# nerfstudio-project/gsplat

Hardware: AMD Instinct MI355X
Metric: Mpixels/s fwd+bwd @1M Gaussians/1080p (higher is better)
Workload: dtype f32; 1 GPU; c3: 1M synthetic Gaussians, 1x1920x1080, SH deg 3, 16x16 tiles, fwd+bwd; gaussians_per_gpu=1000000, cameras_per_gpu=1, packed=False, parallelism=single

## Files before the change

gsplat_amd/csrc/bitonic64.hpp:

```cpp
#pragma once
#include "common.hpp"

namespace gsx {

constexpr uint64_t kBtPadInt = ~0ull;
constexpr uint64_t kBtPadF64 = 0x7FF0000000000000ull;

__device__ __forceinline__ int bt_phys(int i) { return i + (i >> 3); }
__device__ __forceinline__ int bt_off(int b, int lj)
{
    const int sb = b << lj;
    return sb + (sb >> 3);
}
__device__ __forceinline__ bool bt_key_is_odd(uint32_t depth_bits)
{
    return (depth_bits - 0x00100000u) >= (0x7FF00000u - 0x00100000u);
}

__device__ __forceinline__ void bt_cmpx_int(uint64_t &x, uint64_t &y, bool up)
{
    const bool sw     = (x > y) == up;
    const uint64_t lo = sw ? y : x, hi = sw ? x : y;
    x = lo;
    y = hi;
}
__device__ __forceinline__ void bt_cmpx_int_up(uint64_t &x, uint64_t &y)
{
    const bool sw    = x > y;
    const uint64_t t = sw ? y : x;
    y                = sw ? x : y;
    x                = t;
}

template <int G, int NT>
__device__ __forceinline__ void bt_group_int(uint64_t *s, int P, int lk, int lj, int tid)
{
    constexpr int R = 1 << G;
    for (int t = tid; t < (P >> G); t += NT) {
        const int i = ((t >> lj) << (lj + G)) | (t & ((1 << lj) - 1));
        const uint32_t m32 = 0u - (((uint32_t)i >> lk) & 1u);
        const uint64_t m   = ((uint64_t)m32 << 32) | m32;
        uint64_t *p        = s + bt_phys(i);
        uint64_t e[R];
#pragma unroll
        for (int b = 0; b < R; ++b) e[b] = p[bt_off(b, lj)] ^ m;
#pragma unroll
        for (int q = G - 1; q >= 0; --q)
#pragma unroll
            for (int b = 0; b < R; ++b)
                if (!(b & (1 << q))) bt_cmpx_int_up(e[b], e[b | (1 << q)]);
#pragma unroll
        for (int b = 0; b < R; ++b) p[bt_off(b, lj)] = e[b] ^ m;
    }
}

template <int NT, typename Sync>
__device__ __forceinline__ void bt_sort_int(uint64_t *s, int lp, int tid, Sync &&SYNC)
{
    const int P = 1 << lp;
    for (int t = tid; t < (P >> 3); t += NT) {
        uint64_t *p = s + 9 * t;
        uint64_t e[8];
#pragma unroll
        for (int b = 0; b < 8; ++b) e[b] = p[b];
#pragma unroll
        for (int lk = 1; lk <= 3; ++lk)
#pragma unroll
            for (int q = lk - 1; q >= 0; --q)
#pragma unroll
                for (int b = 0; b < 8; ++b)
                    if (!(b & (1 << q))) {
                        const bool up = lk < 3 ? ((b & (1 << lk)) == 0) : ((t & 1) == 0);
                        bt_cmpx_int(e[b], e[b | (1 << q)], up);
                    }
#pragma unroll
        for (int b = 0; b < 8; ++b) p[b] = e[b];
    }
    SYNC();
    for (int lk = 4; lk <= lp; ++lk) {
        for (int top = lk - 1; top >= 0;) {
            const int gsz = top + 1 < 3 ? top + 1 : 3;
            const int lj  = top - gsz + 1;
            if (gsz == 3) bt_group_int<3, NT>(s, P, lk, lj, tid);
            else if (gsz == 2) bt_group_int<2, NT>(s, P, lk, lj, tid);
            else bt_group_int<1, NT>(s, P, lk, lj, tid);
            SYNC();
            top -= gsz;
        }
    }
}

__device__ __forceinline__ void bt_minmax(double &x, double &y)
{
    double lo, hi;
    asm("v_min_f64 %0, %1, %2" : "=v"(lo) : "v"(x), "v"(y));
    asm("v_max_f64 %0, %1, %2" : "=v"(hi) : "v"(x), "v"(y));
    x = lo;
    y = hi;
}
__device__ __forceinline__ double bt_as_f64(uint64_t w) { return __builtin_bit_cast(double, w); }
__device__ __forceinline__ uint64_t bt_as_u64(double d) { return __builtin_bit_cast(uint64_t, d); }

template <int G, int NT>
__device__ __forceinline__ void bt_group_f64(uint64_t *s, int P, int lk, int lj, int tid)
{
    constexpr int R = 1 << G;
    for (int t = tid; t < (P >> G); t += NT) {
        const int i = ((t >> lj) << (lj + G)) | (t & ((1 << lj) - 1));
        const uint64_t neg = (uint64_t)(((uint32_t)i >> lk) & 1u) << 63;
        uint64_t *p        = s + bt_phys(i);
        double e[R];
#pragma unroll
        for (int b = 0; b < R; ++b) e[b] = bt_as_f64(p[bt_off(b, lj)] ^ neg);
#pragma unroll
        for (int q = G - 1; q >= 0; --q)
#pragma unroll
            for (int b = 0; b < R; ++b)
                if (!(b & (1 << q))) bt_minmax(e[b], e[b | (1 << q)]);
#pragma unroll
        for (int b = 0; b < R; ++b) p[bt_off(b, lj)] = bt_as_u64(e[b]) ^ neg;
    }
}

template <int NT, typename Sync>
__device__ __forceinline__ void bt_sort_f64(uint64_t *s, int lp, int tid, Sync &&SYNC)
{
    const int P = 1 << lp;
    for (int t = tid; t < (P >> 3); t += NT) {
        uint64_t *p = s + 9 * t;
        double e[8];
#pragma unroll
        for (int b = 0; b < 8; ++b) e[b] = bt_as_f64(p[b]);
#pragma unroll
        for (int lk = 1; lk <= 2; ++lk)
#pragma unroll
            for (int q = lk - 1; q >= 0; --q)
#pragma unroll
                for (int b = 0; b < 8; ++b)
                    if (!(b & (1 << q))) {
                        if ((b & (1 << lk)) == 0) bt_minmax(e[b], e[b | (1 << q)]);
                        else bt_minmax(e[b | (1 << q)], e[b]);
                    }
        const uint64_t neg = (uint64_t)((uint32_t)t & 1u) << 63;
#pragma unroll
        for (int b = 0; b < 8; ++b) e[b] = bt_as_f64(bt_as_u64(e[b]) ^ neg);
#pragma unroll
        for (int q = 2; q >= 0; --q)
#pragma unroll
            for (int b = 0; b < 8; ++b)
                if (!(b & (1 << q))) bt_minmax(e[b], e[b | (1 << q)]);
#pragma unroll
        for (int b = 0; b < 8; ++b) p[b] = bt_as_u64(e[b]) ^ neg;
    }
    SYNC();
    for (int lk = 4; lk <= lp; ++lk) {
        for (int top = lk - 1; top >= 0;) {
            const int gsz = top + 1 < 3 ? top + 1 : 3;
            const int lj  = top - gsz + 1;
            if (gsz == 3) bt_group_f64<3, NT>(s, P, lk, lj, tid);
            else if (gsz == 2) bt_group_f64<2, NT>(s, P, lk, lj, tid);
            else bt_group_f64<1, NT>(s, P, lk, lj, tid);
            SYNC();
            top -= gsz;
        }
    }
}

bool bitonic_f64_enabled();

}
```

gsplat_amd/csrc/isect_binned.hip:

```cpp
#include "isect_binwalk.hpp"
#include "bitonic64.hpp"
#include "isect_fused.hpp"
#include <cstdlib>
#include <mutex>
#include <new>

namespace gsx {

constexpr int kRowThreads     = 1024;
constexpr int kBnThreads      = 256;
constexpr int kBnMaxBins      = 16384;
constexpr uint32_t kBnMaxTiles = 36864;

struct BinHeader {
    int32_t overflow;
    int32_t big_count;
    int32_t b_done;
    int32_t pad[5];
};

struct BinGeom {
    int64_t rows, rows_per_image, cap_entries;
    uint32_t n_images, cpi, rpc, n_chunks;
    uint32_t tile_size, tile_w, tile_h, n_tiles;
    uint32_t bw, bh, bins_x, bins_y, n_bins, n_bins_total, tile_bits;
    uint32_t kx, ky;
    int32_t skew_cap;
    int32_t skew_ratio;
};

struct BinBuffers {
    BinHeader *hdr;
    int32_t *table;
    int32_t *bin_count;
    int32_t *unit_count;
    uint4 *unit_rec;
    uint32_t *unit_row;
    int32_t *bin_start;
    uint4 *row_rec;
    uint2 *e_pair;
    uint16_t *e_mask;
    int32_t *tile_count;
    int32_t *big_list;
};

struct BinArgs {
    BinGeom g;
    BinBuffers b;
    const float *means2d;
    const int32_t *radii;
    const float *depths;
    const float *conics;
    const float *opacities;
    const uint8_t *tile_mask;
    int32_t *tiles_per_gauss;
    int32_t *isect_offsets;
    int64_t *n_isects;
    int64_t *max_tile_len;
    uint64_t *keys_out;
    int32_t *vals_out;
    uint2 *bucketed;
    uint32_t dbg;
    uint32_t sort_int;
};

__device__ __forceinline__ void bn_chunk_rows(const BinGeom &g, uint32_t chunk, int64_t &lo, int64_t &hi, uint32_t &img)
{
    img                = chunk / g.cpi;
    const uint32_t sub = chunk % g.cpi;
    lo                 = (int64_t)img * g.rows_per_image + (int64_t)sub * g.rpc;
    hi                 = min(lo + (int64_t)g.rpc, (int64_t)(img + 1) * g.rows_per_image);
}

struct BnRow {
    float mx, my, rx, ry, A, B, C, op;
};
__device__ __forceinline__ BnRow bn_load_row(const BinArgs &a, int64_t r, bool has_conic)
{
    BnRow q;
    const int2 rad = reinterpret_cast<const int2 *>(a.radii)[r];
    const v2f m    = reinterpret_cast<const v2f *>(a.means2d)[r];
    q.rx = (float)rad.x; q.ry = (float)rad.y; q.mx = m.x; q.my = m.y;
    q.A = q.B = q.C = q.op = 0.0f;
    if (has_conic) {
        q.A  = a.conics[3 * r];
        q.B  = a.conics[3 * r + 1];
        q.C  = a.conics[3 * r + 2];
        q.op = a.opacities[r];
    }
    return q;
}
__device__ __forceinline__ WalkPrep bn_prepare(const BnRow &q, bool has_conic, const BinGeom &g)
{
    if (!(q.rx > 0.0f && q.ry > 0.0f)) {
        WalkPrep p{};
        p.any = false;
        return p;
    }
    return walk_prepare(q.mx, q.my, q.rx, q.ry, has_conic, q.A, q.B, q.C, q.op, g.tile_size, g.tile_w, g.tile_h);
}

constexpr uint32_t kRecNone = 0u, kRecSmall = 1u, kRecBig = 2u;
constexpr int kInlineSlabs  = 2;
constexpr int kAPark        = 512;
constexpr int kAQueue       = 2048;
constexpr int kATake        = 128;
constexpr int kParkWords    = 17;
constexpr uint32_t kUnitCap = 1024;

template <bool FIXED>
struct BinShape {
    uint32_t bw, bh, kx, ky;
    __device__ __forceinline__ explicit BinShape(const BinGeom &g)
        : bw(FIXED ? 4u : g.bw), bh(FIXED ? 2u : g.bh), kx(FIXED ? 2u : g.kx), ky(FIXED ? 4u : g.ky) {}
};
template <bool FIXED>
__device__ __forceinline__ uint32_t rec_bin_mask(uint64_t M, const BinShape<FIXED> &sh, uint32_t i, uint32_t j)
{
    return block_bin_mask(M, sh.bw, sh.bh, sh.kx, i, j);
}
template <bool FIXED>
__device__ __forceinline__ uint4 make_record(uint64_t M, uint32_t bbx, uint32_t bby, uint32_t dbits, const BinGeom &g,
                                             const BinShape<FIXED> &sh, int32_t *s_hist)
{
    uint32_t used = 0;
    for (uint32_t j = 0; j < sh.ky; ++j)
        for (uint32_t i = 0; i < sh.kx; ++i)
            if (rec_bin_mask(M, sh, i, j)) {
                used |= 1u << (j * sh.kx + i);
                if (s_hist) atomicAdd(&s_hist[(bby + j) * g.bins_x + bbx + i], 1);
            }
    return make_uint4((uint32_t)M, (uint32_t)(M >> 32), bbx | (bby << 8) | (kRecSmall << 16) | (used << 18), dbits);
}

__device__ __forceinline__ void park_walk(uint32_t *rw, const WalkPrep &p, uint32_t slot, bool one, uint32_t org, uint32_t dbits)
{
    rw[0] = (uint32_t)p.x0 | ((uint32_t)p.y0 << 16); rw[1] = (uint32_t)p.x1 | ((uint32_t)p.y1 << 16);
    rw[2] = slot | (p.ellipse ? 1u << 16 : 0u) | (p.alongY ? 1u << 17 : 0u) | (one ? 1u << 18 : 0u);
    rw[3] = org;
    rw[4] = dbits;
    const float pf[12] = {p.B, p.coeff, p.disc, p.t, p.pu, p.pv, p.bmin_u, p.bmax_u, p.bmin_v, p.bmax_v, p.u_at_vmin, p.u_at_vmax};
#pragma unroll
    for (int k = 0; k < 12; ++k) rw[5 + k] = __float_as_uint(pf[k]);
}
__device__ __forceinline__ WalkPrep parked_walk(const uint32_t *rw)
{
    WalkPrep p;
    p.x0 = (int)(rw[0] & 0xFFFFu); p.y0 = (int)(rw[0] >> 16); p.x1 = (int)(rw[1] & 0xFFFFu); p.y1 = (int)(rw[1] >> 16);
    p.any = true; p.ellipse = (rw[2] >> 16) & 1u; p.alongY = (rw[2] >> 17) & 1u;
    p.B = __uint_as_float(rw[5]); p.coeff = __uint_as_float(rw[6]); p.disc = __uint_as_float(rw[7]);
    p.t = __uint_as_float(rw[8]); p.pu = __uint_as_float(rw[9]); p.pv = __uint_as_float(rw[10]);
    p.bmin_u = __uint_as_float(rw[11]); p.bmax_u = __uint_as_float(rw[12]); p.bmin_v = __uint_as_float(rw[13]);
    p.bmax_v = __uint_as_float(rw[14]); p.u_at_vmin = __uint_as_float(rw[15]); p.u_at_vmax = __uint_as_float(rw[16]);
    return p;
}

template <bool FIXED>
__global__ void __launch_bounds__(kRowThreads) bin_rect_kernel(const BinArgs a)
{
    extern __shared__ int32_t s_hist[];
    __shared__ uint32_t s_q[kAQueue];
    __shared__ uint32_t s_row[kAPark][kParkWords];
    __shared__ int32_t s_tpg[2 * kRowThreads];
    __shared__ int32_t s_qn, s_qlim, s_mn, s_units, s_anybig;
    const BinGeom &g = a.g;
    const BinShape<FIXED> sh(g);
    for (uint32_t i = threadIdx.x; i < g.n_bins; i += kRowThreads) s_hist[i] = 0;
    if (threadIdx.x == 0) {
        s_units = 0; s_mn = 0; s_qn = 0; s_qlim = kAQueue; s_anybig = 0;
        if (blockIdx.x == 0) { a.b.hdr->overflow = 0; a.b.hdr->big_count = 0; a.b.hdr->b_done = 0; }
    }
    int64_t lo, hi;
    uint32_t img;
    bn_chunk_rows(g, blockIdx.x, lo, hi, img);
    const bool has_conic = (a.conics != nullptr) && (a.opacities != nullptr);
    const uint8_t *tmask = a.tile_mask ? a.tile_mask + (size_t)img * g.n_tiles : nullptr;
    const uint32_t W = sh.kx * sh.bw, Hh = sh.ky * sh.bh;
    uint64_t col = 0;
    for (uint32_t y = 0; y < Hh; ++y) col |= 1ull << (y * W);
    uint4 *unit_rec    = a.b.unit_rec + (size_t)blockIdx.x * kUnitCap;
    uint32_t *unit_row = a.b.unit_row + (size_t)blockIdx.x * kUnitCap;
    constexpr int kU = 2;
    for (int64_t base = lo; base < hi; base += kRowThreads * kU) {
        BnRow q[kU];
        uint32_t dbits[kU];
#pragma unroll
        for (int u = 0; u < kU; ++u) {
            const int64_t r = base + u * kRowThreads + threadIdx.x;
            q[u].rx = q[u].ry = 0.0f;
            dbits[u] = 0u;
            if (r < hi) {
                q[u]     = bn_load_row(a, r, has_conic);
                dbits[u] = __float_as_uint(a.depths[r]);
            }
        }
        if (base != lo) {
            __syncthreads();
            if (threadIdx.x == 0) { s_mn = 0; s_qn = 0; s_qlim = kAQueue; s_anybig = 0; }
        }
        __syncthreads();
        uint32_t units[kU], done[kU];
        int32_t ms[kU];
        bool left = false;
#pragma unroll
        for (int u = 0; u < kU; ++u) {
            const int64_t r = base + u * kRowThreads + threadIdx.x;
            units[u] = done[u] = 0u;
            ms[u]    = -1;
            if (r >= hi) continue;
            uint4 rec        = make_uint4(0u, 0u, kRecNone << 16, dbits[u]);
            const WalkPrep p = bn_prepare(q[u], has_conic, g);
            bool now         = true;
            if (p.any) {
                const uint32_t bx0 = (uint32_t)p.x0 / sh.bw, bx1 = ((uint32_t)p.x1 + sh.bw - 1) / sh.bw;
                const uint32_t by0 = (uint32_t)p.y0 / sh.bh, by1 = ((uint32_t)p.y1 + sh.bh - 1) / sh.bh;
                const uint32_t w = bx1 - bx0, h = by1 - by0;
                const bool one   = w <= sh.kx && h <= sh.ky;
                const int slabs  = p.ellipse ? min(p.x1 - p.x0, p.y1 - p.y0) : 1;
                if (one && slabs <= (int)(((a.dbg >> 16) & 15u) ? ((a.dbg >> 16) & 15u) : (uint32_t)kInlineSlabs) && !(a.dbg & 16u)) {
                    const int cx0 = (int)(bx0 * sh.bw), cy0 = (int)(by0 * sh.bh);
                    rec = make_record(block_mask(p, g.tile_size, g.tile_w, cx0, cy0, cx0 + (int)W, cy0 + (int)Hh, W, col, tmask), bx0, by0, dbits[u], g, sh, s_hist);
                } else if (!(a.dbg & 64u)) {
                    units[u] = one ? 1u : ((w + sh.kx - 1) / sh.kx) * ((h + sh.ky - 1) / sh.ky);
                    const int32_t m = atomicAdd(&s_mn, 1);
                    if (m < kAPark) {
                        ms[u] = m;
                        park_walk(s_row[m], p, (uint32_t)(u * kRowThreads) + threadIdx.x, one,
                                  bx0 | (by0 << 8) | ((w - 1u) << 16) | ((h - 1u) << 24), dbits[u]);
                        const int32_t take = (int32_t)min(units[u], (uint32_t)kATake);
                        const int32_t qpos = atomicAdd(&s_qn, take);
                        if (qpos + take > kAQueue) atomicMin(&s_qlim, qpos);
                        else {
                            for (int32_t k = 0; k < take; ++k) s_q[qpos + k] = (uint32_t)m | ((uint32_t)k << 9);
                            done[u] = (uint32_t)take;
                        }
                    }
                    left |= done[u] != units[u];
                    if (one) now = false;
                    else {
                        rec.z = kRecBig << 16;
                        s_tpg[u * kRowThreads + threadIdx.x] = 0;
                        s_anybig = 1;
                    }
                }
            }
            if (now && !(a.dbg & 32u)) {
                a.b.row_rec[r] = rec;
                if (a.tiles_per_gauss && ((rec.z >> 16) & 3u) != kRecBig) a.tiles_per_gauss[r] = __popc(rec.x) + __popc(rec.y);
            }
        }
        for (bool more = __syncthreads_or(left);;) {
            const int32_t n_q = (a.dbg & 256u) ? 0 : min(s_qn, s_qlim);
            for (int32_t k = (int32_t)threadIdx.x; k < n_q; k += kRowThreads) {
                const uint32_t pr  = s_q[k];
                const uint32_t *rw = s_row[pr & 511u];
                const WalkPrep p   = parked_walk(rw);
                const int slot     = (int)(rw[2] & 0xFFFFu);
                const bool one     = (rw[2] >> 18) & 1u;
                const uint32_t o = rw[3], bx0 = o & 255u, by0 = (o >> 8) & 255u, w = ((o >> 16) & 255u) + 1u;
                const uint32_t wb = (w + sh.kx - 1) / sh.kx, idx = pr >> 9;
                const uint32_t bbx = bx0 + (idx % wb) * sh.kx, bby = by0 + (idx / wb) * sh.ky;
                const int cx0 = (int)(bbx * sh.bw), cy0 = (int)(bby * sh.bh);
                const uint64_t M = (a.dbg & 512u) ? 1ull : block_mask(p, g.tile_size, g.tile_w, cx0, cy0, cx0 + (int)W, cy0 + (int)Hh, W, col, tmask);
                const int64_t r  = base + slot;
                if (one) {
                    a.b.row_rec[r] = make_record(M, bbx, bby, rw[4], g, sh, s_hist);
                    if (a.tiles_per_gauss) a.tiles_per_gauss[r] = __popcll(M);
                } else if (M) {
                    const uint32_t at = (uint32_t)atomicAdd(&s_units, 1);
                    const uint4 rec   = make_record(M, bbx, bby, rw[4], g, sh, s_hist);
                    if (at < kUnitCap) {
                        unit_rec[at] = rec;
                        unit_row[at] = (uint32_t)r;
                    }
                    atomicAdd(&s_tpg[slot], __popcll(M));
                }
            }
            if (!more) break;
            __syncthreads();
            if (threadIdx.x == 0) { s_mn = 0; s_qn = 0; s_qlim = kAQueue; }
            __syncthreads();
            left = false;
#pragma unroll
            for (int u = 0; u < kU; ++u) {
                if (units[u] == done[u]) continue;
                const int32_t m = atomicAdd(&s_mn, 1);
                if (m < kAPark) {
                    const int64_t r  = base + u * kRowThreads + threadIdx.x;
                    const WalkPrep p = bn_prepare(bn_load_row(a, r, has_conic), has_conic, g);
                    const uint32_t bx0 = (uint32_t)p.x0 / sh.bw, bx1 = ((uint32_t)p.x1 + sh.bw - 1) / sh.bw;
                    const uint32_t by0 = (uint32_t)p.y0 / sh.bh, by1 = ((uint32_t)p.y1 + sh.bh - 1) / sh.bh;
                    park_walk(s_row[m], p, (uint32_t)(u * kRowThreads) + threadIdx.x, units[u] == 1u,
                              bx0 | (by0 << 8) | ((bx1 - bx0 - 1u) << 16) | ((by1 - by0 - 1u) << 24), dbits[u]);
                    const int32_t take = (int32_t)min(units[u] - done[u], (uint32_t)kATake);
                    const int32_t qpos = atomicAdd(&s_qn, take);
                    if (qpos + take > kAQueue) atomicMin(&s_qlim, qpos);
                    else {
                        for (int32_t k = 0; k < take; ++k) s_q[qpos + k] = (uint32_t)m | ((done[u] + (uint32_t)k) << 9);
                        done[u] += (uint32_t)take;
                    }
                }
                left |= done[u] != units[u];
            }
            more = __syncthreads_or(left);
        }
        if (s_anybig) {
            __syncthreads();
            if (a.tiles_per_gauss) {
#pragma unroll
                for (int u = 0; u < kU; ++u) {
                    const int64_t r = base + u * kRowThreads + threadIdx.x;
                    if (r < hi && units[u] > 1u) a.tiles_per_gauss[r] = s_tpg[u * kRowThreads + threadIdx.x];
                }
            }
        }
    }
    __syncthreads();
    int32_t *out = a.b.table + (int64_t)blockIdx.x * g.n_bins;
    for (uint32_t i = threadIdx.x; i < g.n_bins; i += kRowThreads) out[i] = s_hist[i];
    if (threadIdx.x == 0) a.b.unit_count[blockIdx.x] = s_units;
}

constexpr int kCsCols = 32, kCsSegs2 = 32, kCsPer = 32;
__global__ void __launch_bounds__(kCsCols *kCsSegs2) bin_colscan_kernel(const BinArgs a, uint32_t col_groups)
{
    __shared__ int32_t s_seg[kCsSegs2][kCsCols + 1];
    __shared__ int64_t s_part[16];
    __shared__ int32_t s_max, s_last, s_umax[16];
    const BinGeom &g      = a.g;
    const uint32_t n_cols = g.n_bins, cpi = g.cpi;
    const uint32_t img = blockIdx.x / col_groups, cg = blockIdx.x % col_groups;
    const uint32_t lane_c = threadIdx.x % kCsCols, seg = threadIdx.x / kCsCols;
    const uint32_t c      = cg * kCsCols + lane_c;
    const bool live       = c < n_cols;
    const uint32_t per    = (cpi + kCsSegs2 - 1) / kCsSegs2;
    const uint32_t r0 = seg * per, r1 = min(r0 + per, cpi);
    int32_t *col = a.b.table + (int64_t)img * cpi * n_cols + c;
    int32_t v[kCsPer];
    int32_t sum = 0;
#pragma unroll
    for (int i = 0; i < kCsPer; ++i) {
        const uint32_t r = r0 + (uint32_t)i;
        v[i]             = (live && r < r1) ? col[(int64_t)r * n_cols] : 0;
    }
#pragma unroll
    for (int i = 0; i < kCsPer; ++i) sum += v[i];
    s_seg[seg][lane_c] = sum;
    __syncthreads();
    int32_t run = 0;
    for (uint32_t k = 0; k < seg; ++k) run += s_seg[k][lane_c];
    if (live) {
#pragma unroll
        for (int i = 0; i < kCsPer; ++i) {
            const uint32_t r = r0 + (uint32_t)i;
            if (r < r1) col[(int64_t)r * n_cols] = run;
            run += v[i];
        }
        if (seg == kCsSegs2 - 1) a.b.bin_count[(int64_t)img * n_cols + c] = run;
    }
    __syncthreads();
    if (threadIdx.x == 0)
        s_last = __hip_atomic_fetch_add(&a.b.hdr->b_done, 1, __ATOMIC_RELEASE, __HIP_MEMORY_SCOPE_AGENT) == (int32_t)gridDim.x - 1;
    __syncthreads();
    if (!s_last) return;
    __builtin_amdgcn_fence(__ATOMIC_ACQUIRE, "agent");
    const int64_t n = block_scan_i32_1024(a.b.bin_count, a.b.bin_start, g.n_bins_total, s_part, &s_max);
    int32_t um = 0;
    for (uint32_t i = threadIdx.x; i < g.n_chunks; i += kCsCols * kCsSegs2) um = max(um, a.b.unit_count[i]);
    um = wave_max_i32(um);
    if ((threadIdx.x & 63u) == 0) s_umax[threadIdx.x >> 6] = um;
    __syncthreads();
    if (threadIdx.x == 0) {
        for (int w = 1; w < 16; ++w) um = max(um, s_umax[w]);
        const int64_t mx    = s_max;
        const bool lopsided = g.skew_ratio > 0 && mx * (int64_t)g.n_bins_total > (int64_t)g.skew_ratio * n && mx > 256;
        a.b.bin_start[g.n_bins_total] = (int32_t)min(n, (int64_t)INT32_MAX);
        a.b.hdr->overflow = (n > g.cap_entries || um > (int32_t)kUnitCap || (g.skew_cap > 0 && mx > g.skew_cap) || lopsided) ? 1 : 0;
    }
}

template <bool FIXED>
__device__ __forceinline__ void bn_deal(const BinArgs &a, const BinShape<FIXED> &sh, const uint4 &rec, uint32_t row, int32_t *s_cur)
{
    const uint32_t bx0 = rec.z & 255u, by0 = (rec.z >> 8) & 255u;
    const uint64_t M   = ((uint64_t)rec.y << 32) | rec.x;
    for (uint32_t used = rec.z >> 18; used;) {
        const uint32_t k = (uint32_t)__builtin_ctz(used);
        used &= used - 1u;
        const uint32_t i = k % sh.kx, j = k / sh.kx;
        const int32_t slot = atomicAdd(&s_cur[(by0 + j) * a.g.bins_x + bx0 + i], 1);
        if (a.dbg & 8u) continue;
        a.b.e_pair[slot] = make_uint2(rec.w, row);
        a.b.e_mask[slot] = (uint16_t)rec_bin_mask(M, sh, i, j);
    }
}

template <bool FIXED>
__global__ void __launch_bounds__(kRowThreads) bin_scatter_kernel(const BinArgs a)
{
    extern __shared__ int32_t s_cur[];
    const BinGeom &g = a.g;
    const BinShape<FIXED> sh(g);
    const uint32_t per_xcd = gridDim.x / 8u;
    const uint32_t chunk   = (a.dbg & 4096u) ? blockIdx.x : (blockIdx.x % 8u) * per_xcd + blockIdx.x / 8u;
    if (chunk >= g.n_chunks) return;
    int64_t lo, hi;
    uint32_t img;
    bn_chunk_rows(g, chunk, lo, hi, img);
    constexpr int kU = 2;
    uint4 rec[kU];
#pragma unroll
    for (int u = 0; u < kU; ++u) {
        const int64_t r = lo + u * kRowThreads + threadIdx.x;
        rec[u]          = r < hi ? a.b.row_rec[r] : make_uint4(0u, 0u, 0u, 0u);
    }
    const int32_t *start = a.b.bin_start + (int64_t)img * g.n_bins;
    const int32_t *pre   = a.b.table + (int64_t)chunk * g.n_bins;
    for (uint32_t i = threadIdx.x; i < g.n_bins; i += kRowThreads) s_cur[i] = start[i] + pre[i];
    const int32_t n_units = min(a.b.unit_count[chunk], (int32_t)kUnitCap);
    if (a.b.hdr->overflow) return;
    __syncthreads();
    for (int64_t base = lo; base < hi; base += kU * kRowThreads) {
#pragma unroll
        for (int u = 0; u < kU; ++u) {
            const int64_t r = base + u * kRowThreads + threadIdx.x;
            if (base != lo) rec[u] = r < hi ? a.b.row_rec[r] : make_uint4(0u, 0u, 0u, 0u);
            if (((rec[u].z >> 16) & 3u) == kRecSmall) bn_deal(a, sh, rec[u], (uint32_t)r, s_cur);
        }
    }
    for (int32_t k = (int32_t)threadIdx.x; k < n_units; k += kRowThreads)
        bn_deal(a, sh, a.b.unit_rec[(size_t)chunk * kUnitCap + k], a.b.unit_row[(size_t)chunk * kUnitCap + k], s_cur);
}

__global__ void __launch_bounds__(kBnThreads) bin_tiles_kernel(const BinArgs a)
{
    __shared__ int32_t s_cnt[16];
    const BinGeom &g = a.g;
    if (a.b.hdr->overflow) return;
    const uint32_t bin = blockIdx.x;
    const int32_t e0 = a.b.bin_start[bin], e1 = a.b.bin_start[bin + 1];
    const int lane = (int)(threadIdx.x & 63u);
    const int n_bits = (int)(g.bw * g.bh);
    if (threadIdx.x < 16) s_cnt[threadIdx.x] = 0;
    __syncthreads();
    int32_t mine = 0;
    constexpr int kU = 8;
    for (int32_t base = e0; base < e1; base += kBnThreads * kU) {
        uint32_t m[kU];
#pragma unroll
        for (int u = 0; u < kU; ++u) {
            const int32_t e = base + u * kBnThreads + (int32_t)threadIdx.x;
            m[u]            = e < e1 ? (uint32_t)a.b.e_mask[e] : 0u;
        }
#pragma unroll
        for (int u = 0; u < kU; ++u) {
            if (base + u * kBnThreads >= e1) break;
            for (int t = 0; t < n_bits; ++t) {
                const uint64_t b = __builtin_amdgcn_ballot_w64((m[u] >> t) & 1u);
                if (lane == t) mine += (int32_t)__popcll(b);
            }
        }
    }
    if (lane < n_bits && mine) atomicAdd(&s_cnt[lane], mine);
    __syncthreads();
    if ((int)threadIdx.x < n_bits) {
        const uint32_t img = bin / g.n_bins, lb = bin % g.n_bins;
        const uint32_t tx = (lb % g.bins_x) * g.bw + threadIdx.x % g.bw, ty = (lb / g.bins_x) * g.bh + threadIdx.x / g.bw;
        if (tx < g.tile_w && ty < g.tile_h) a.b.tile_count[(size_t)img * g.n_tiles + (size_t)ty * g.tile_w + tx] = s_cnt[threadIdx.x];
    }
}

__global__ void __launch_bounds__(1024) tile_plan_kernel(const BinArgs a)
{
    __shared__ int64_t s_part[16];
    __shared__ int32_t s_max;
    const BinGeom &g = a.g;
    if (a.b.hdr->overflow) {
        if (threadIdx.x == 0) {
            __threadfence_system();
            *a.n_isects = GSX_ISECT_RETRY;
        }
        return;
    }
    const uint32_t nt   = g.n_images * g.n_tiles;
    const int64_t total = block_scan_i32_1024(a.b.tile_count, a.isect_offsets, nt, s_part, a.max_tile_len ? &s_max : nullptr);
    if (threadIdx.x == 0) {
        if (a.max_tile_len) *a.max_tile_len = (int64_t)s_max;
        __threadfence_system();
        *a.n_isects = total;
    }
}

constexpr int kArenaPerWave = 512;

__global__ void __launch_bounds__(1024) bin_sort_kernel(const BinArgs a)
{
    extern __shared__ __attribute__((aligned(16))) unsigned char smem_raw[];
    const BinGeom &g = a.g;
    const int n_bits = (int)(g.bw * g.bh), n_thr = n_bits * 64;
    const int arena_words = kArenaPerWave * n_bits;
    uint64_t *s_arena = reinterpret_cast<uint64_t *>(smem_raw);
    __shared__ int32_t s_tcnt[16], s_goff[16], s_base[16], s_batch[16], s_cur[16], s_nbatch, s_n;
    __shared__ uint32_t s_odd;
    __shared__ uint64_t s_hi[16];
    const uint32_t bin = blockIdx.x;
    const int32_t e0 = a.b.bin_start[bin], e1 = a.b.bin_start[bin + 1];
    if (e0 == e1) return;
    const uint32_t img = bin / g.n_bins, lb = bin % g.n_bins;
    const uint32_t tx0 = (lb % g.bins_x) * g.bw, ty0 = (lb / g.bins_x) * g.bh;
    const int lane = (int)(threadIdx.x & 63u), wave = (int)(threadIdx.x >> 6);
    const uint64_t lt_mask = (lane == 0) ? 0ull : (~0ull >> (64 - lane));
    if ((int)threadIdx.x < 16) {
        const int t       = (int)threadIdx.x;
        const uint32_t tx = tx0 + (uint32_t)t % g.bw, ty = ty0 + (uint32_t)t / g.bw;
        const bool in     = t < n_bits && tx < g.tile_w && ty < g.tile_h;
        const size_t gid  = (size_t)img * g.n_tiles + (size_t)ty * g.tile_w + tx;
        const int n       = in ? a.b.tile_count[gid] : 0;
        s_tcnt[t]         = n;
        s_goff[t]         = in ? a.isect_offsets[gid] : 0;
        s_hi[t]           = in ? ((((uint64_t)img << g.tile_bits) | ((uint64_t)ty * g.tile_w + tx)) << 32) : 0ull;
        int P = 0;
        if (n > 0) {
            P = 64;
            while (P < n) P <<= 1;
        }
        const bool big = P > arena_words;
        if (big) P = 0;
        int batch = 0, used = 0, my_batch = n > 0 ? 0 : -1, my_base = 0;
        for (int k = 0; k < 16; ++k) {
            const int Pk = __shfl(P, k, 16);
            if (Pk == 0) continue;
            if (used + Pk > arena_words) { ++batch; used = 0; }
            if (k == t) { my_batch = batch; my_base = used + (used >> 3); }
            used += Pk;
        }
        s_batch[t] = big ? -2 : my_batch;
        s_base[t]  = my_base;
        if (t == 15) s_nbatch = batch + 1;
    }
    __syncthreads();
    const int n_batch = s_nbatch;
    for (int b = 0; b < n_batch; ++b) {
        if (threadIdx.x < 16) s_cur[threadIdx.x] = 0;
        if (threadIdx.x == 16) s_odd = a.sort_int ? 0xFFFFu : 0u;
        uint32_t bmask = 0;
        for (int t = 0; t < n_bits; ++t) bmask |= (s_batch[t] == b) ? (1u << t) : 0u;
        __syncthreads();
        for (int32_t e = e0 + (int32_t)threadIdx.x; e < e1 && !(a.dbg & 2u); e += n_thr) {
            uint32_t m = (uint32_t)a.b.e_mask[e] & bmask;
            if (m == 0u) continue;
            const uint2 pr     = a.b.e_pair[e];
            const uint64_t key = ((uint64_t)pr.x << 32) | pr.y;
            if (bt_key_is_odd(pr.x)) atomicOr(&s_odd, m);
            while (m) {
                const int t = __builtin_ctz(m);
                m &= m - 1u;
                const int32_t pos = atomicAdd(&s_cur[t], 1);
                s_arena[s_base[t] + bt_phys(pos)] = key;
            }
        }
        __syncthreads();
        if (wave < n_bits && s_batch[wave] == b) {
            uint64_t *sw = s_arena + s_base[wave];
            const int n  = s_tcnt[wave];
            int lp = 6;
            while ((1 << lp) < n) ++lp;
            const bool as_int = (s_odd >> wave) & 1u;
            const uint64_t pad = as_int ? kBtPadInt : kBtPadF64;
            for (int i = n + lane; i < (1 << lp); i += 64) sw[bt_phys(i)] = pad;
            wave_lds_sync();
            if (a.dbg & 1u) {
            } else if (as_int) bt_sort_int<64>(sw, lp, lane, [] { wave_lds_sync(); });
            else bt_sort_f64<64>(sw, lp, lane, [] { wave_lds_sync(); });
            const int64_t off = s_goff[wave];
            const uint64_t hi = s_hi[wave];
            for (int i = lane; i < n; i += 64) {
                const uint64_t w    = sw[bt_phys(i)];
                a.keys_out[off + i] = hi | (w >> 32);
                a.vals_out[off + i] = (int32_t)(uint32_t)w;
            }
        }
        __syncthreads();
    }
    for (int t = 0; t < n_bits; ++t) {
        if (s_batch[t] != -2) continue;
        if (threadIdx.x == 0) s_n = 0;
        __syncthreads();
        const int64_t off = s_goff[t];
        for (int32_t base = e0; base < e1; base += n_thr) {
            const int32_t e    = base + (int32_t)threadIdx.x;
            const bool has     = e < e1 && (((uint32_t)a.b.e_mask[e] >> t) & 1u);
            const uint64_t bal = __builtin_amdgcn_ballot_w64(has);
            if (bal == 0ull) continue;
            const int first = (int)__builtin_ctzll(bal);
            int32_t wbase   = 0;
            if (lane == first) wbase = atomicAdd(&s_n, (int32_t)__popcll(bal));
            wbase = __builtin_amdgcn_readlane(wbase, first);
            if (has) a.bucketed[off + wbase + (int32_t)__popcll(bal & lt_mask)] = a.b.e_pair[e];
        }
        if (threadIdx.x == 0) {
            const uint32_t tx = tx0 + (uint32_t)t % g.bw, ty = ty0 + (uint32_t)t / g.bw;
            a.b.big_list[atomicAdd(&a.b.hdr->big_count, 1)] = (int32_t)(img * g.n_tiles + ty * g.tile_w + tx);
        }
        __syncthreads();
    }
}

static int64_t align256(int64_t x) { return (x + 255) & ~(int64_t)255; }
static uint32_t bits_for(uint64_t count)
{
    uint32_t b = 0;
    if (count <= 1) return 0;
    uint64_t v = count - 1;
    while (v) { ++b; v >>= 1; }
    return b;
}

static void bin_dims(uint32_t &bw, uint32_t &bh)
{
    bw = 4; bh = 2;
    if (const char *e = getenv("GSX_ISECT_BIN")) {
        unsigned w = 0, h = 0;
        if (sscanf(e, "%ux%u", &w, &h) == 2 && w >= 1 && h >= 1 && w * h <= 16) { bw = w; bh = h; }
    }
}

static bool bin_geometry(BinGeom &g, int64_t rows, uint32_t n_images, uint32_t tile_size, uint32_t tile_w, uint32_t tile_h,
                         int64_t cap_entries)
{
    g = BinGeom{};
    g.rows = rows; g.n_images = n_images ? n_images : 1;
    g.rows_per_image = rows / g.n_images;
    bin_dims(g.bw, g.bh);
    g.tile_size = tile_size; g.tile_w = tile_w; g.tile_h = tile_h; g.n_tiles = tile_w * tile_h;
    g.bins_x = (tile_w + g.bw - 1) / g.bw; g.bins_y = (tile_h + g.bh - 1) / g.bh;
    g.kx = 2; g.ky = g.bw * g.bh <= 8 ? 4 : 2;
    g.n_bins = g.bins_x * g.bins_y; g.n_bins_total = g.n_bins * g.n_images;
    g.tile_bits = bits_for(g.n_tiles);
    const int64_t max_cpi = 1024 / g.n_images > 0 ? 1024 / g.n_images : 1;
    int64_t cpi = (g.rows_per_image + 2047) / 2048;
    {
        const int64_t per_image = (256 + (int64_t)g.n_images - 1) / (int64_t)g.n_images;
        const int64_t floor_cpi = g.rows_per_image / 1024 < per_image ? g.rows_per_image / 1024 : per_image;
        if (cpi < floor_cpi) cpi = floor_cpi;
    }
    if (cpi < 1) cpi = 1;
    if (cpi > max_cpi) cpi = max_cpi;
    g.cpi = (uint32_t)cpi;
    g.rpc = (uint32_t)((g.rows_per_image + cpi - 1) / cpi);
    if (g.rpc == 0) g.rpc = 1;
    g.n_chunks    = g.cpi * g.n_images;
    g.cap_entries = cap_entries;
    return g.n_bins_total <= (uint32_t)kBnMaxBins && (uint64_t)g.n_images * g.n_tiles <= kBnMaxTiles && rows < (1ll << 28)
           && g.bins_x <= 256 && g.bins_y <= 256;
}

static int64_t bin_cap_entries(int64_t rows) { return 4 * rows + 262144; }

static int64_t bin_layout(const BinGeom &g, unsigned char *base, BinBuffers *b)
{
    unsigned char *p = base;
    auto take = [&](int64_t bytes) {
        unsigned char *q = p;
        p += align256(bytes);
        return q;
    };
    BinBuffers t{};
    t.hdr        = reinterpret_cast<BinHeader *>(take(sizeof(BinHeader)));
    t.table      = reinterpret_cast<int32_t *>(take((int64_t)g.n_chunks * g.n_bins * 4));
    t.bin_count  = reinterpret_cast<int32_t *>(take((int64_t)g.n_bins_total * 4));
    t.unit_count = reinterpret_cast<int32_t *>(take((int64_t)g.n_chunks * 4));
    t.unit_rec   = reinterpret_cast<uint4 *>(take((int64_t)g.n_chunks * kUnitCap * 16));
    t.unit_row   = reinterpret_cast<uint32_t *>(take((int64_t)g.n_chunks * kUnitCap * 4));
    t.bin_start  = reinterpret_cast<int32_t *>(take(((int64_t)g.n_bins_total + 1) * 4));
    t.row_rec    = reinterpret_cast<uint4 *>(take(g.rows * 16));
    t.e_pair     = reinterpret_cast<uint2 *>(take(g.cap_entries * 8));
    t.e_mask     = reinterpret_cast<uint16_t *>(take(g.cap_entries * 2));
    t.tile_count = reinterpret_cast<int32_t *>(take((int64_t)g.n_images * g.n_tiles * 4));
    t.big_list   = reinterpret_cast<int32_t *>(take((int64_t)g.n_images * g.n_tiles * 4));
    if (b) *b = t;
    return (int64_t)(p - base);
}

}

using namespace gsx;

namespace {
struct RetryNote { uint64_t key; int left; };
struct PathMemory {
    std::mutex mu;
    RetryNote notes[16] = {};
    uint32_t next = 0;
};
thread_local PathMemory t_default_memory;
thread_local PathMemory *t_current_memory = nullptr;
PathMemory &current_memory() { return t_current_memory ? *t_current_memory : t_default_memory; }
uint64_t retry_key(int64_t rows, uint32_t n_images, uint32_t tile_w, uint32_t tile_h)
{
    return ((uint64_t)(rows >> 16) << 40) ^ ((uint64_t)n_images << 32) ^ ((uint64_t)tile_w << 16) ^ (uint64_t)tile_h ^ (1ull << 63);
}
bool retried_recently(int64_t rows, uint32_t n_images, uint32_t tile_w, uint32_t tile_h, bool consume)
{
    const uint64_t key = retry_key(rows, n_images, tile_w, tile_h);
    PathMemory &m = current_memory();
    std::lock_guard<std::mutex> lock(m.mu);
    for (auto &n : m.notes)
        if (n.key == key && n.left > 0) {
            if (consume) --n.left;
            return true;
        }
    return false;
}
}

extern "C" void *gsx_isect_path_memory_create(void) { return new (std::nothrow) PathMemory(); }
extern "C" void gsx_isect_path_memory_destroy(void *mem)
{
    PathMemory *m = static_cast<PathMemory *>(mem);
    if (m && t_current_memory == m) t_current_memory = nullptr;
    delete m;
}
extern "C" void *gsx_isect_path_memory_use(void *mem)
{
    void *prev = t_current_memory;
    t_current_memory = static_cast<PathMemory *>(mem);
    return prev;
}

extern "C" int gsx_isect_binned_note_retry(int64_t rows, uint32_t n_images, uint32_t tile_w, uint32_t tile_h)
{
    const uint64_t key = retry_key(rows, n_images, tile_w, tile_h);
    PathMemory &m = current_memory();
    std::lock_guard<std::mutex> lock(m.mu);
    for (auto &n : m.notes)
        if (n.key == key) {
            n.left = 63;
            return GSX_OK;
        }
    m.notes[m.next++ % 16u] = RetryNote{key, 63};
    return GSX_OK;
}

static int binned_decide(int64_t rows, uint32_t n_images, uint32_t tile_w, uint32_t tile_h, int packed, bool consume);
extern "C" int gsx_isect_binned_supported(int64_t rows, uint32_t n_images, uint32_t tile_w, uint32_t tile_h, int packed)
{
    return binned_decide(rows, n_images, tile_w, tile_h, packed, false);
}
extern "C" int gsx_isect_binned_should_try(int64_t rows, uint32_t n_images, uint32_t tile_w, uint32_t tile_h, int packed)
{
    return binned_decide(rows, n_images, tile_w, tile_h, packed, true);
}
static int binned_decide(int64_t rows, uint32_t n_images, uint32_t tile_w, uint32_t tile_h, int packed, bool consume)
{
    const char *force = getenv("GSX_ISECT_PATH");
    if (getenv("GSX_ISECT_LEGACY") || (force && force[0] == 'l')) return 0;
    if (packed && n_images != 1) return 0;
    if (n_images < 1 || tile_w < 1 || tile_h < 1 || rows < 0) return 0;
    if (rows % n_images != 0) return 0;
    BinGeom g;
    if (!bin_geometry(g, rows > 0 ? rows : 1, n_images, 16, tile_w, tile_h, 1)) return 0;
    if (force && force[0] == 'b') return 1;
    if (!(g.rows_per_image >= 49152 && g.rows_per_image <= 144ll * (int64_t)g.n_tiles)) return 0;
    return retried_recently(rows, n_images, tile_w, tile_h, consume) ? 0 : 1;
}

extern "C" int64_t gsx_isect_binned_count_workspace_bytes(int64_t rows, uint32_t n_images, uint32_t tile_w, uint32_t tile_h)
{
    BinGeom g;
    if (rows < 1) rows = 1;
    bin_geometry(g, rows, n_images, 16, tile_w, tile_h, bin_cap_entries(rows));
    return bin_layout(g, nullptr, nullptr) + 512;
}

extern "C" int64_t gsx_isect_binned_emit_workspace_bytes(int64_t n_isects)
{
    if (n_isects < 1) n_isects = 1;
    return 2 * align256(n_isects * 8) + 512;
}

static int binned_setup(const char *fn, BinArgs &a, int64_t rows, uint32_t n_images, uint32_t tile_size, uint32_t tile_w,
                        uint32_t tile_h, void *ws, int64_t ws_bytes)
{
    GSX_REQUIRE(rows >= 1 && tile_size > 0, "%s: bad rows / tile_size", fn);
    GSX_REQUIRE(rows % (n_images ? n_images : 1) == 0, "%s: rows (%lld) must be a multiple of n_images (%u)", fn,
                (long long)rows, n_images);
    GSX_REQUIRE(bin_geometry(a.g, rows, n_images, tile_size, tile_w, tile_h, bin_cap_entries(rows)),
                "%s: %u images x %u x %u tiles not supported", fn, n_images, tile_w, tile_h);
    if (const char *e = getenv("GSX_ISECT_DBG")) a.dbg = (uint32_t)atoi(e);
    a.sort_int = bitonic_f64_enabled() ? 0u : 1u;
    {
        const char *force = getenv("GSX_ISECT_PATH"), *sk = getenv("GSX_ISECT_BIN_SKEW");
        a.g.skew_cap = (force && force[0] == 'b') ? 0 : (int32_t)(kArenaPerWave * (int)(a.g.bw * a.g.bh) * 3 / 4);
        a.g.skew_ratio = (force && force[0] == 'b') ? 0 : 4;
        if (sk) { a.g.skew_cap = atoi(sk); a.g.skew_ratio = a.g.skew_cap > 0 ? 4 : 0; }
    }
    unsigned char *base = reinterpret_cast<unsigned char *>((reinterpret_cast<uintptr_t>(ws) + 255) & ~(uintptr_t)255);
    if (ws == nullptr || (base - reinterpret_cast<unsigned char *>(ws)) + bin_layout(a.g, base, &a.b) > ws_bytes) {
        set_last_error("%s: count workspace too small", fn);
        return GSX_ERR_WORKSPACE;
    }
    return GSX_OK;
}

extern "C" int gsx_isect_binned_count(const float *means2d, const int32_t *radii, const float *depths, const float *conics,
                                      const float *opacities, const uint8_t *tile_mask, int64_t rows, uint32_t n_images,
                                      uint32_t tile_size, uint32_t tile_w, uint32_t tile_h, int32_t *tiles_per_gauss,
                                      int32_t *isect_offsets, int64_t *n_isects, int64_t *max_tile_len, void *count_workspace,
                                      int64_t count_workspace_bytes, void *stream)
{
    hipStream_t s = (hipStream_t)stream;
    const uint32_t n_bins = n_images * tile_w * tile_h;
    GSX_REQUIRE(isect_offsets && n_isects, "gsx_isect_binned_count: null output");
    if (rows == 0) {
        if (max_tile_len && hipMemsetAsync(max_tile_len, 0, 8, s) != hipSuccess) return check_launch("isect_binned_count memset");
        if (hipMemsetAsync(isect_offsets, 0, (size_t)n_bins * 4, s) != hipSuccess
            || hipMemsetAsync(n_isects, 0, 8, s) != hipSuccess) {
            set_last_error("gsx_isect_binned_count: memset failed");
            return GSX_ERR_LAUNCH;
        }
        return GSX_OK;
    }
    GSX_REQUIRE(means2d && radii && depths, "gsx_isect_binned_count: null pointer");
    BinArgs a{};
    int rc = binned_setup("gsx_isect_binned_count", a, rows, n_images, tile_size, tile_w, tile_h, count_workspace,
                          count_workspace_bytes);
    if (rc != GSX_OK) return rc;
    a.means2d = means2d; a.radii = radii; a.depths = depths; a.conics = conics; a.opacities = opacities;
    a.tile_mask = tile_mask; a.tiles_per_gauss = tiles_per_gauss; a.isect_offsets = isect_offsets; a.n_isects = n_isects;
    a.max_tile_len = max_tile_len;
    const size_t bins_lds = (size_t)a.g.n_bins * sizeof(int32_t);
    const bool fixed      = a.g.bw == 4 && a.g.bh == 2 && a.g.kx == 2 && a.g.ky == 4;
    static PerDeviceOnce once;
    if (once.first()) {
        (void)hipFuncSetAttribute((const void *)bin_rect_kernel<true>, hipFuncAttributeMaxDynamicSharedMemorySize, 64 * 1024);
        (void)hipFuncSetAttribute((const void *)bin_rect_kernel<false>, hipFuncAttributeMaxDynamicSharedMemorySize, 64 * 1024);
    }
    if (fixed) bin_rect_kernel<true><<<dim3(a.g.n_chunks), dim3(kRowThreads), bins_lds, s>>>(a);
    else bin_rect_kernel<false><<<dim3(a.g.n_chunks), dim3(kRowThreads), bins_lds, s>>>(a);
    const uint32_t col_groups = (a.g.n_bins + kCsCols - 1) / kCsCols;
    bin_colscan_kernel<<<dim3(col_groups * a.g.n_images), dim3(kCsCols * kCsSegs2), 0, s>>>(a, col_groups);
    const uint32_t d_grid = (a.g.n_chunks + 7u) / 8u * 8u;
    if (fixed) bin_scatter_kernel<true><<<dim3(d_grid), dim3(kRowThreads), bins_lds, s>>>(a);
    else bin_scatter_kernel<false><<<dim3(d_grid), dim3(kRowThreads), bins_lds, s>>>(a);
    bin_tiles_kernel<<<dim3(a.g.n_bins_total), dim3(kBnThreads), 0, s>>>(a);
    tile_plan_kernel<<<dim3(1), dim3(1024), 0, s>>>(a);
    return check_launch("isect_binned_count");
}

extern "C" int gsx_isect_binned_emit_sort(int64_t rows, uint32_t n_images, uint32_t tile_size, uint32_t tile_w,
                                          uint32_t tile_h, void *count_workspace, int64_t count_workspace_bytes,
                                          const int32_t *isect_offsets, int64_t n_isects, int64_t longest_list,
                                          int64_t *isect_ids_sorted, int32_t *flatten_ids_sorted, void *workspace,
                                          int64_t workspace_bytes, void *stream)
{
    GSX_REQUIRE(n_isects >= 0 && n_isects < (1ll << 31), "gsx_isect_binned_emit_sort: n_isects out of range");
    if (n_isects == 0 || rows == 0) return GSX_OK;
    GSX_REQUIRE(isect_offsets && isect_ids_sorted && flatten_ids_sorted, "gsx_isect_binned_emit_sort: null pointer");
    hipStream_t s = (hipStream_t)stream;
    BinArgs a{};
    int rc = binned_setup("gsx_isect_binned_emit_sort", a, rows, n_images, tile_size, tile_w, tile_h, count_workspace,
                          count_workspace_bytes);
    if (rc != GSX_OK) return rc;
    if (workspace == nullptr || workspace_bytes < gsx_isect_binned_emit_workspace_bytes(n_isects)) {
        set_last_error("gsx_isect_binned_emit_sort: workspace too small");
        return GSX_ERR_WORKSPACE;
    }
    unsigned char *p = reinterpret_cast<unsigned char *>((reinterpret_cast<uintptr_t>(workspace) + 255) & ~(uintptr_t)255);
    a.bucketed = reinterpret_cast<uint2 *>(p); p += align256(n_isects * 8);
    uint2 *scratch = reinterpret_cast<uint2 *>(p);
    a.isect_offsets = const_cast<int32_t *>(isect_offsets);
    a.keys_out = reinterpret_cast<uint64_t *>(isect_ids_sorted);
    a.vals_out = flatten_ids_sorted;
    const int n_bits = (int)(a.g.bw * a.g.bh);
    const size_t sort_lds = (size_t)(kArenaPerWave * n_bits) * 9;
    static PerDeviceOnce once;
    if (once.first())
        (void)hipFuncSetAttribute((const void *)bin_sort_kernel, hipFuncAttributeMaxDynamicSharedMemorySize, 112 * 1024);
    bin_sort_kernel<<<dim3(a.g.n_bins_total), dim3(64 * n_bits), sort_lds, s>>>(a);
    rc = check_launch("isect_binned_emit");
    if (rc != GSX_OK) return rc;
    TileSortArgs t{};
    t.n = n_isects; t.n_tiles = a.g.n_tiles; t.tile_bits = a.g.tile_bits; t.n_bins = a.g.n_images * a.g.n_tiles;
    t.n_chunks = 1;
    t.table_scanned = const_cast<int32_t *>(isect_offsets);
    t.bucketed = a.bucketed; t.scratch = scratch;
    t.big_count = &a.b.hdr->big_count; t.big_list = a.b.big_list;
    t.keys_out = a.keys_out; t.vals_out = a.vals_out;
    if (longest_list > 0 && longest_list <= (int64_t)(kArenaPerWave * n_bits) / 2) return GSX_OK;
    return launch_big_tile_sort(t, s);
}
```

Before: 2333 Mpixels/s.

## Sort per-tile f64 keys in registers with cross-lane DPP/permlane bitonic network

For tiles with up to 512 float-orderable keys, each lane loads 8 keys into registers and runs the whole bitonic sort using DPP and permlane16/32 swaps for the cross-lane stages. Lanes are mapped to register groups through a bit permutation. This replaces the LDS-based group passes and their wave syncs with register exchanges. It also sets amdgpu_waves_per_eu(8) on the bin sort kernel, which constrains register use and may cause spills.

```diff
diff --git a/gsplat_amd/csrc/bitonic64.hpp b/gsplat_amd/csrc/bitonic64.hpp
--- a/gsplat_amd/csrc/bitonic64.hpp
+++ b/gsplat_amd/csrc/bitonic64.hpp
@@ -166,6 +166,112 @@
     }
 }
 
+__host__ __device__ constexpr int bt_lane_bit(int b) { return b == 0 ? 4 : b == 1 ? 5 : b == 2 ? 0 : b == 3 ? 1 : b == 4 ? 3 : 2; }
+__device__ __forceinline__ int bt_reg_group(int lane)
+{
+    int g = 0;
+#pragma unroll
+    for (int b = 0; b < 6; ++b) g |= ((lane >> bt_lane_bit(b)) & 1) << b;
+    return g;
+}
+
+template <int CTRL>
+__device__ __forceinline__ double bt_dpp_f64(double x)
+{
+    const uint64_t u  = bt_as_u64(x);
+    const int lo      = (int)(uint32_t)u, hi = (int)(uint32_t)(u >> 32);
+    const uint32_t l2 = (uint32_t)__builtin_amdgcn_update_dpp(lo, lo, CTRL, 0xF, 0xF, true);
+    const uint32_t h2 = (uint32_t)__builtin_amdgcn_update_dpp(hi, hi, CTRL, 0xF, 0xF, true);
+    return bt_as_f64(((uint64_t)h2 << 32) | l2);
+}
+
+template <int LB>
+__device__ __forceinline__ void bt_xlane(double (&e)[8], int lane)
+{
+    if constexpr (LB >= 4) {
+#pragma unroll
+        for (int q = 0; q < 4; ++q) {
+            const uint64_t a = bt_as_u64(e[2 * q]), b = bt_as_u64(e[2 * q + 1]);
+            auto swp = [](uint32_t x, uint32_t y) {
+                if constexpr (LB == 4) return __builtin_amdgcn_permlane16_swap(x, y, false, false);
+                else return __builtin_amdgcn_permlane32_swap(x, y, false, false);
+            };
+            const auto l = swp((uint32_t)a, (uint32_t)b), h = swp((uint32_t)(a >> 32), (uint32_t)(b >> 32));
+            double x = bt_as_f64(((uint64_t)h[0] << 32) | l[0]), y = bt_as_f64(((uint64_t)h[1] << 32) | l[1]);
+            bt_minmax(x, y);
+            const uint64_t u = bt_as_u64(x), v = bt_as_u64(y);
+            const auto l2 = swp((uint32_t)u, (uint32_t)v), h2 = swp((uint32_t)(u >> 32), (uint32_t)(v >> 32));
+            e[2 * q]     = bt_as_f64(((uint64_t)h2[0] << 32) | l2[0]);
+            e[2 * q + 1] = bt_as_f64(((uint64_t)h2[1] << 32) | l2[1]);
+        }
+    } else {
+        const bool low = ((lane >> LB) & 1) == 0;
+#pragma unroll
+        for (int r = 0; r < 8; ++r) {
+            double p;
+            if constexpr (LB == 0) p = bt_dpp_f64<0xB1>(e[r]);
+            else if constexpr (LB == 1) p = bt_dpp_f64<0x4E>(e[r]);
+            else if constexpr (LB == 2) p = bt_dpp_f64<0x141>(bt_dpp_f64<0x1B>(e[r]));
+            else p = bt_dpp_f64<0x128>(e[r]);
+            double lo = e[r], hi = p;
+            bt_minmax(lo, hi);
+            e[r] = low ? lo : hi;
+        }
+    }
+}
+
+template <int LJ>
+__device__ __forceinline__ void bt_xlane_stages(double (&e)[8], int lane)
+{
+    if constexpr (LJ >= 3) {
+        bt_xlane<bt_lane_bit(LJ - 3)>(e, lane);
+        bt_xlane_stages<LJ - 1>(e, lane);
+    }
+}
+
+__device__ __forceinline__ void bt_reg_stages(double (&e)[8])
+{
+#pragma unroll
+    for (int q = 2; q >= 0; --q)
+#pragma unroll
+        for (int b = 0; b < 8; ++b)
+            if (!(b & (1 << q))) bt_minmax(e[b], e[b | (1 << q)]);
+}
+
+template <int LK>
+__device__ __forceinline__ void bt_phase_regs(double (&e)[8], int lane)
+{
+    uint64_t neg = 0;
+    if constexpr (LK < 9) neg = (uint64_t)((lane >> bt_lane_bit(LK - 3)) & 1) << 63;
+#pragma unroll
+    for (int r = 0; r < 8; ++r) e[r] = bt_as_f64(bt_as_u64(e[r]) ^ neg);
+    bt_xlane_stages<LK - 1>(e, lane);
+    bt_reg_stages(e);
+#pragma unroll
+    for (int r = 0; r < 8; ++r) e[r] = bt_as_f64(bt_as_u64(e[r]) ^ neg);
+}
+
+__device__ __forceinline__ void bt_sort_f64_regs(double (&e)[8], int lp, int lane)
+{
+#pragma unroll
+    for (int lk = 1; lk <= 2; ++lk)
+#pragma unroll
+        for (int q = lk - 1; q >= 0; --q)
+#pragma unroll
+            for (int b = 0; b < 8; ++b)
+                if (!(b & (1 << q))) {
+                    if ((b & (1 << lk)) == 0) bt_minmax(e[b], e[b | (1 << q)]);
+                    else bt_minmax(e[b | (1 << q)], e[b]);
+                }
+    bt_phase_regs<3>(e, lane);
+    bt_phase_regs<4>(e, lane);
+    bt_phase_regs<5>(e, lane);
+    bt_phase_regs<6>(e, lane);
+    if (lp >= 7) bt_phase_regs<7>(e, lane);
+    if (lp >= 8) bt_phase_regs<8>(e, lane);
+    if (lp >= 9) bt_phase_regs<9>(e, lane);
+}
+
 bool bitonic_f64_enabled();
 
 }
diff --git a/gsplat_amd/csrc/isect_binned.hip b/gsplat_amd/csrc/isect_binned.hip
--- a/gsplat_amd/csrc/isect_binned.hip
+++ b/gsplat_amd/csrc/isect_binned.hip
@@ -493,7 +493,7 @@
 
 constexpr int kArenaPerWave = 512;
 
-__global__ void __launch_bounds__(1024) bin_sort_kernel(const BinArgs a)
+__global__ void __launch_bounds__(1024) __attribute__((amdgpu_waves_per_eu(8))) bin_sort_kernel(const BinArgs a)
 {
     extern __shared__ __attribute__((aligned(16))) unsigned char smem_raw[];
     const BinGeom &g = a.g;
@@ -566,12 +566,24 @@
             int lp = 6;
             while ((1 << lp) < n) ++lp;
             const bool as_int = (s_odd >> wave) & 1u;
-            const uint64_t pad = as_int ? kBtPadInt : kBtPadF64;
-            for (int i = n + lane; i < (1 << lp); i += 64) sw[bt_phys(i)] = pad;
+            if (!as_int && lp <= 9 && !(a.dbg & 1u)) {
+                const int grp = bt_reg_group(lane);
+                double e[8];
+#pragma unroll
+                for (int r = 0; r < 8; ++r) e[r] = bt_as_f64(8 * grp + r < n ? sw[9 * grp + r] : kBtPadF64);
+                bt_sort_f64_regs(e, lp, lane);
+#pragma unroll
+                for (int r = 0; r < 8; ++r)
+                    if (8 * grp + r < n) sw[9 * grp + r] = bt_as_u64(e[r]);
+            } else {
+                const uint64_t pad = as_int ? kBtPadInt : kBtPadF64;
+                for (int i = n + lane; i < (1 << lp); i += 64) sw[bt_phys(i)] = pad;
+                wave_lds_sync();
+                if (a.dbg & 1u) {
+                } else if (as_int) bt_sort_int<64>(sw, lp, lane, [] { wave_lds_sync(); });
+                else bt_sort_f64<64>(sw, lp, lane, [] { wave_lds_sync(); });
+            }
             wave_lds_sync();
-            if (a.dbg & 1u) {
-            } else if (as_int) bt_sort_int<64>(sw, lp, lane, [] { wave_lds_sync(); });
-            else bt_sort_f64<64>(sw, lp, lane, [] { wave_lds_sync(); });
             const int64_t off = s_goff[wave];
             const uint64_t hi = s_hi[wave];
             for (int i = lane; i < n; i += 64) {
```

Result: no change. 2335 Mpixels/s (median of 5 runs) (+0.1%).
